# littlemesie/recommend-tf2.0

Measured on NVIDIA B200. Metric: DLRM train samples/sec, higher is better.
Workload: dtype f32

## Files before the change

### include/rtf_b200.h

```cpp
#ifndef RTF_B200_H
#define RTF_B200_H

#include <stddef.h>
#include <stdint.h>

#ifdef __cplusplus
extern "C" {
#endif

#define RTF_MAX_FIELDS 64

#define RTF_E_ARG (-1)
#define RTF_E_ALIGN (-2)
#define RTF_E_RANGE (-3)
#define RTF_E_WORKSPACE (-4)

enum { RTF_POOL_NONE = 0, RTF_POOL_SUM = 1, RTF_POOL_MEAN = 2,
       RTF_POOL_SKIP_INVALID = 0x100 };
enum { RTF_OPT_NONE = 0, RTF_OPT_SGD = 1, RTF_OPT_ADAGRAD = 2, RTF_OPT_ADAM = 3 };

typedef struct rtf_opt {
  int32_t kind;
  float lr;
  float beta1;
// ... 116 lines not shown
int rtf_din_attn_bwd(const float* d_q, int64_t q_sb, const float* d_k, int64_t k_sb,
                     const float* d_v, int64_t v_sb, const float* d_mask, int64_t m_sb,
                     const float* d_W, const float* d_bias, int act, int64_t B, int L, int d,
                     const float* d_gout, int64_t go_sb, float* d_gq, int64_t gq_sb, float* d_gk,
                     int64_t gk_sb, float* d_gv, int64_t gv_sb, float* d_gw_rows, void* stream);

int rtf_log_uniform_workspace(int S, size_t* bytes);
int rtf_log_uniform_sample(uint64_t seed, int S, int64_t range_max, int64_t* d_sampled,
                           int32_t* d_num_tries, void* d_ws, void* stream);
int rtf_log_uniform_sample_dseed(const uint64_t* d_seed, int S, int64_t range_max,
                                 int64_t* d_sampled, int32_t* d_num_tries, void* d_ws, void* stream);
int rtf_log_uniform_expected(const int64_t* d_ids, int64_t n, int64_t range_max,
                             const int32_t* d_num_tries, float* d_out, void* stream);
int rtf_sampled_softmax_workspace(int S, int D, size_t* bytes);
int rtf_sampled_softmax_fwd(const float* d_x, int64_t x_sb, const float* d_W, const float* d_bias,
                            const int64_t* d_labels, const int64_t* d_sampled,
                            const float* d_true_exp, const float* d_samp_exp, int64_t B, int64_t N,
                            int S, int D, int remove_hits, float* d_loss, float* d_lse, void* d_ws,
                            int32_t* d_err, void* stream);
int rtf_sampled_softmax_bwd(const float* d_x, int64_t x_sb, const float* d_W, const float* d_bias,
                            const int64_t* d_labels, const int64_t* d_sampled,
                            const float* d_true_exp, const float* d_samp_exp, int64_t B, int64_t N,
                            int S, int D, int remove_hits, const float* d_lse,
                            const float* d_gloss, float* d_gx, int64_t gx_sb, float* d_G,
                            void* d_ws, void* stream);

int rtf_ssm_gather(const float* d_W, const float* d_bias, const int64_t* d_sampled,
                   const float* d_samp_exp, int64_t N, int S, int D, float* d_Ws, float* d_cs,
                   int32_t* d_err, void* stream);
int rtf_ssm_logits_fwd(const float* d_logits, int64_t ld, const float* d_x, int64_t x_sb,
                       const float* d_W, const float* d_bias, const int64_t* d_labels,
                       const int64_t* d_sampled, const float* d_true_exp, const float* d_cs,
                       int64_t B, int64_t N, int S, int D, int remove_hits, float* d_loss,
                       float* d_lse, int32_t* d_err, void* stream);
int rtf_ssm_logits_bwd(const float* d_logits, int64_t ld, const float* d_x, int64_t x_sb,
                       const float* d_W, const float* d_bias, const int64_t* d_labels,
                       const int64_t* d_sampled, const float* d_true_exp, const float* d_cs,
                       int64_t B, int64_t N, int S, int D, int remove_hits, const float* d_lse,
                       const float* d_gloss, float* d_g0, float* d_G1, int64_t g1_ld, void* stream);
int rtf_ssm_true_gx(const float* d_W, const int64_t* d_labels, const float* d_g0, int64_t B,
                    int64_t N, int D, float* d_gx, int64_t gx_sb, void* stream);

int rtf_relu_bwd_colsum_workspace(int64_t B, int cols, size_t* bytes);
int rtf_relu_bwd_colsum(const float* d_gy, const float* d_y, int64_t B, int cols, float* d_g,
                        float* d_colsum, void* d_ws, void* stream);

int rtf_bce_workspace(int64_t n, size_t* bytes);
int rtf_bce_fwd(const float* d_y, const float* d_p, int64_t n, float* d_loss, float* d_dp,
                void* d_ws, void* stream);

int rtf_bn_workspace(int64_t B, int C, size_t* bytes);
int rtf_bn_fwd(const float* d_x, int64_t ldx, int64_t B, int C, const float* d_gamma,
               const float* d_beta, float eps, float momentum, float* d_y, int64_t ldy,
               float* d_mean, float* d_invstd, float* d_moving_mean, float* d_moving_var,
               void* d_ws, size_t ws_bytes, void* stream);
int rtf_bn_bwd(const float* d_dy, int64_t lddy, const float* d_x, int64_t ldx, int64_t B, int C,
               const float* d_mean, const float* d_invstd, const float* d_gamma, float* d_dx,
               int64_t lddx, float* d_dgamma, float* d_dbeta, void* d_ws, size_t ws_bytes,
               void* stream);

int rtf_layernorm_workspace(int64_t rows, int C, size_t* bytes);
int rtf_layernorm_fwd(const float* d_x, int64_t rows, int C, const float* d_gamma,
                      const float* d_beta, float eps, float* d_y, float* d_mean, float* d_rstd,
                      void* stream);
int rtf_layernorm_bwd(const float* d_dy, const float* d_x, const float* d_mean, const float* d_rstd,
                      const float* d_gamma, int64_t rows, int C, float* d_dx, float* d_dgamma,
                      float* d_dbeta, void* d_ws, size_t ws_bytes, void* stream);

int rtf_dense_gemm_nn_workspace(int M, int N, int K, int batch, size_t* bytes);
int rtf_dense_gemm_nt_workspace(int M, int N, int K, int batch, size_t* bytes);
int rtf_dense_gemm_tn_workspace(int M, int N, int K, int batch, size_t* bytes);
int rtf_dense_gemm_nn(const float* d_a, int64_t lda, int64_t stride_a, const float* d_b, int64_t ldb,
                      int64_t stride_b, const float* d_bias, int relu, float* d_out, int64_t ldd,
                      int64_t stride_d, int M, int N, int K, int batch, void* d_ws, size_t ws_bytes,
                      void* stream);
int rtf_dense_gemm_nt(const float* d_a, int64_t lda, int64_t stride_a, const float* d_b, int64_t ldb,
                      int64_t stride_b, const float* d_bias, int relu, float* d_out, int64_t ldd,
                      int64_t stride_d, int M, int N, int K, int batch, void* d_ws, size_t ws_bytes,
                      void* stream);
int rtf_dense_gemm_tn(const float* d_a, int64_t lda, int64_t stride_a, const float* d_b, int64_t ldb,
                      int64_t stride_b, const float* d_bias, int relu, float* d_out, int64_t ldd,
                      int64_t stride_d, int M, int N, int K, int batch, void* d_ws, size_t ws_bytes,
                      void* stream);

int rtf_autoint_layer_supported(int F, int dm, int H, int hs);
int rtf_autoint_layer_workspace(int64_t B, int dm, int HS, size_t* bytes);
int rtf_autoint_layer_fwd(const float* d_x, int64_t B, int F, int dm, const float* d_wq,
                          const float* d_wk, const float* d_wv, const float* d_w0, int H, int hs,
                          int act, float scale, float* d_out, void* stream);
int rtf_autoint_layer_bwd(const float* d_x, int64_t B, int F, int dm, const float* d_wq,
                          const float* d_wk, const float* d_wv, const float* d_w0, int H, int hs,
                          int act, float scale, const float* d_out, const float* d_gout,
                          float* d_gx, float* d_gw, void* d_ws, size_t ws_bytes, void* stream);

int rtf_sasrec_score_fwd(const float* d_info, int64_t info_sb, const float* d_pos_tab,
                         int64_t pos_rows, const float* d_neg_tab, int64_t neg_rows,
                         const void* d_pos_ids, const void* d_neg_ids, int ids_i64, int64_t neg_sb,
                         int64_t B, int NEG, int D, float* d_logits, float* d_loss_rows,
                         int32_t* d_err, void* stream);
int rtf_sasrec_score_bwd(const float* d_info, int64_t info_sb, const float* d_pos_tab,
                         int64_t pos_rows, const float* d_neg_tab, int64_t neg_rows,
                         const void* d_pos_ids, const void* d_neg_ids, int ids_i64, int64_t neg_sb,
                         int64_t B, int NEG, int D, const float* d_logits, const float* d_gloss,
                         const float* d_glogits, float* d_ginfo, float* d_gemb, void* stream);

int rtf_topk_ip_workspace(int64_t B, int64_t N, int D, int k, size_t* bytes);
int rtf_topk_ip(const float* d_users, int64_t u_ld, int64_t B, const float* d_items, int64_t i_ld,
                int64_t N, int D, int k, int64_t* d_out_idx, float* d_out_score, int32_t* d_flag,
                void* d_ws, size_t ws_bytes, void* stream);

int rtf_peer_pull_rows(const int64_t* d_peer_tab, const int64_t* d_peer_str, int64_t sample0, int G,
                       uint64_t rw_mask, const int64_t* rows, int n_fields, int D, const void* d_ids,
                       int ids_i64, int64_t B, int64_t ids_sb, int64_t ids_sf, float* d_out,
                       int64_t out_sb, int32_t* d_err, void* stream);

int rtf_dense_adam(float* d_w, const float* d_g, float* d_m, float* d_v, int64_t n,
                   const rtf_opt* opt, void* stream);
int rtf_rows_apply_dense(float* d_w, float* d_s1, float* d_s2, const float* d_g,
                         const float* d_touched, int64_t rows, int dim, const rtf_opt* opt,
                         void* stream);

#ifdef __cplusplus
}
#endif
#endif
```

### recommend-tf2.0_b200/_lib.py

```python
from __future__ import annotations

import ctypes as C
import os
import subprocess
import sys

_HERE = os.path.dirname(os.path.abspath(__file__))
LIB_PATH = os.path.join(_HERE, "librtf_b200.so")
CSRC_DIR = os.path.join(_HERE, "csrc")
HEADER_PATH = os.path.join(os.path.dirname(_HERE), "include", "rtf_b200.h")

POOL_NONE, POOL_SUM, POOL_MEAN = 0, 1, 2
OPT_NONE, OPT_SGD, OPT_ADAGRAD, OPT_ADAM = 0, 1, 2, 3
SEG_CHUNK = 64
MAX_FIELDS = 64


class RtfError(RuntimeError):
    pass


class rtf_opt(C.Structure):
    _fields_ = [("kind", C.c_int32), ("lr", C.c_float), ("beta1", C.c_float),
                ("beta2", C.c_float), ("eps", C.c_float), ("l2", C.c_float),
                ("lr_dev", C.c_void_p)]


_p = C.c_void_p
_i64 = C.c_int64
_int = C.c_int

SIGNATURES = {
    "rtf_version": [C.POINTER(C.c_int)],
    "rtf_embed_fwd": [_p, _p, _p, _int, _p, _int, _i64, _int, _i64, _i64, _i64, _int, _p, _i64,
                      _p, _p],
    "rtf_embed_bwd_workspace": [_i64, _int, C.POINTER(C.c_size_t)],
    "rtf_embed_bwd": [_p, _p, _p, _p, _p, _int, _p, _int, _p, _int, _i64, _int, _i64, _i64,
                      _i64, _int, _p, _i64, C.POINTER(rtf_opt), _p, _p, _p,
                      C.POINTER(C.c_int), _p, C.c_size_t, _p],
    "rtf_embed_bwd_prepare": [_p, _p, _int, _p, _int, _p, _int, _i64, _int, _i64, _i64, _i64, _p,
                              C.POINTER(C.c_int), _p, C.c_size_t, _p],
    "rtf_embed_bwd_apply": [_p, _p, _p, _p, _p, _int, _p, _int, _i64, _int, _int, _p, _i64,
                            C.POINTER(rtf_opt), _p, _p, _p, C.c_size_t, _p],
    "rtf_dot_interact_fwd": [_p, _i64, _int, _int, _p, _i64, _int, _p],
    "rtf_dot_interact_bwd": [_p, _p, _i64, _i64, _int, _int, _p, _p],
    "rtf_dot_rows_fwd": [_p, _p, _int, _int, _i64, _p, _i64, _int, _p, _i64, _p],
    "rtf_dot_rows_bwd": [_p, _p, _int, _int, _i64, _p, _i64, _p, _p, _p],
    "rtf_embed_dot_fwd": [_p, _p, _int, _int, _p, _int, _i64, _i64, _i64, _p, _i64, _p, _i64,
                          _int, _p, _p],
    "rtf_embed_dot_bwd": [_p, _p, _int, _int, _p, _int, _i64, _i64, _i64, _p, _i64, _p, _i64,
                          _p, _i64, _p, _i64, _p],
    "rtf_embed_dot_peer_fwd": [_p, _p, _i64, _int, C.c_uint64, _p, _int, _int, _p, _int, _i64, _i64, _i64, _p,
                               _i64, _p, _i64, _int, _p, _i64, _p, _p],
    "rtf_embed_dot_peer_bwd": [_p, _i64, _p, _int, _int, _p, _int, _i64, _i64, _i64, _p, _i64, _p,
                               _i64, _p, _i64, _p, _p, _int, C.c_uint64, _i64, _p],
    "rtf_colsum_workspace": [_i64, _int, C.POINTER(C.c_size_t)],
    "rtf_colsum": [_p, _i64, _p, _i64, _int, _p, _p, _p],
    "rtf_bn_workspace": [_i64, _int, C.POINTER(C.c_size_t)],
    "rtf_bn_fwd": [_p, _i64, _i64, _int, _p, _p, C.c_float, C.c_float, _p, _i64, _p, _p, _p, _p, _p,
                   C.c_size_t, _p],
    "rtf_bn_bwd": [_p, _i64, _p, _i64, _i64, _int, _p, _p, _p, _p, _i64, _p, _p, _p, C.c_size_t, _p],
    "rtf_layernorm_workspace": [_i64, _int, C.POINTER(C.c_size_t)],
    "rtf_layernorm_fwd": [_p, _i64, _int, _p, _p, C.c_float, _p, _p, _p, _p],
    "rtf_layernorm_bwd": [_p, _p, _p, _p, _p, _i64, _int, _p, _p, _p, _p, C.c_size_t, _p],
    "rtf_bce_workspace": [_i64, C.POINTER(C.c_size_t)],
    "rtf_bce_fwd": [_p, _p, _i64, _p, _p, _p, _p],
    "rtf_relu_bwd_colsum_workspace": [_i64, _int, C.POINTER(C.c_size_t)],
    "rtf_relu_bwd_colsum": [_p, _p, _i64, _int, _p, _p, _p, _p],
    "rtf_autoint_layer_supported": [_int, _int, _int, _int],
    "rtf_autoint_layer_workspace": [_i64, _int, _int, C.POINTER(C.c_size_t)],
    "rtf_autoint_layer_fwd": [_p, _i64, _int, _int, _p, _p, _p, _p, _int, _int, _int, C.c_float, _p, _p],
    "rtf_autoint_layer_bwd": [_p, _i64, _int, _int, _p, _p, _p, _p, _int, _int, _int, C.c_float, _p, _p,
                              _p, _p, _p, C.c_size_t, _p],
    "rtf_sasrec_score_fwd": [_p, _i64, _p, _i64, _p, _i64, _p, _p, _int, _i64, _i64, _int, _int, _p, _p, _p, _p],
    "rtf_sasrec_score_bwd": [_p, _i64, _p, _i64, _p, _i64, _p, _p, _int, _i64, _i64, _int, _int, _p, _p, _p,
                             _p, _p, _p],
    "rtf_topk_ip_workspace": [_i64, _i64, _int, _int, C.POINTER(C.c_size_t)],
    "rtf_topk_ip": [_p, _i64, _i64, _p, _i64, _i64, _int, _int, _p, _p, _p, _p, C.c_size_t, _p],
    "rtf_peer_pull_rows": [_p, _p, _i64, _int, C.c_uint64, _p, _int, _int, _p, _int, _i64, _i64, _i64, _p,
                           _i64, _p, _p],
    "rtf_ssm_gather": [_p, _p, _p, _p, _i64, _int, _int, _p, _p, _p, _p],
    "rtf_ssm_logits_fwd": [_p, _i64, _p, _i64, _p, _p, _p, _p, _p, _p, _i64, _i64, _int, _int, _int, _p, _p,
                           _p, _p],
    "rtf_ssm_logits_bwd": [_p, _i64, _p, _i64, _p, _p, _p, _p, _p, _p, _i64, _i64, _int, _int, _int, _p, _p,
                           _p, _p, _i64, _p],
    "rtf_ssm_true_gx": [_p, _p, _p, _i64, _i64, _int, _p, _i64, _p],
    "rtf_dense_adam": [_p, _p, _p, _p, _i64, C.POINTER(rtf_opt), _p],
    "rtf_rows_apply_dense": [_p, _p, _p, _p, _p, _i64, _int, C.POINTER(rtf_opt), _p],
    "rtf_dense_gemm_nn_workspace": [_int, _int, _int, _int, C.POINTER(C.c_size_t)],
    "rtf_dense_gemm_nt_workspace": [_int, _int, _int, _int, C.POINTER(C.c_size_t)],
    "rtf_dense_gemm_tn_workspace": [_int, _int, _int, _int, C.POINTER(C.c_size_t)],
    "rtf_dense_gemm_nn": [_p, _i64, _i64, _p, _i64, _i64, _p, _int, _p, _i64, _i64, _int, _int, _int,
                          _int, _p, C.c_size_t, _p],
    "rtf_dense_gemm_nt": [_p, _i64, _i64, _p, _i64, _i64, _p, _int, _p, _i64, _i64, _int, _int, _int,
                          _int, _p, C.c_size_t, _p],
    "rtf_dense_gemm_tn": [_p, _i64, _i64, _p, _i64, _i64, _p, _int, _p, _i64, _i64, _int, _int, _int,
                          _int, _p, C.c_size_t, _p],
    "rtf_fm_layer_workspace": [_i64, _int, C.POINTER(C.c_size_t)],
    "rtf_fm_layer_fwd": [_p, _i64, _p, _int, _p, _i64, _int, _int, _i64, _int, _int, _p, _p, _p],
    "rtf_fm_layer_bwd": [_p, _i64, _p, _int, _p, _i64, _int, _int, _i64, _int, _int, _p, _p,
                         _i64, _p, _p, _i64, _p, _p],
    "rtf_fm_gather_fwd": [_p, _p, _int, _int, _int, _p, _int, _p, _i64, _p, _int, _i64, _i64,
                          _i64, _p, _p, _p, _p, _p],
    "rtf_fm_gather_bwd": [_p, _p, _int, _int, _int, _p, _int, _p, _i64, _p, _int, _i64, _i64,
                          _i64, _p, _p, _p, _p, _p, _p, _p],
    "rtf_attn_fwd": [_p, _i64, _i64, _p, _i64, _i64, _p, _i64, _i64, _p, _i64, _p, _i64, _int,
                     _int, _int, _int, _int, _int, C.c_float, _p, _i64, _i64, _p, _p, _p],
    "rtf_attn_bwd": [_p, _i64, _i64, _p, _i64, _i64, _p, _i64, _i64, _p, _i64, _p, _i64, _int,
                     _int, _int, _int, _int, _int, C.c_float, _p, _i64, _i64, _p, _p, _p, _i64,
                     _i64, _p, _p, _i64, _i64, _p, _i64, _i64, _p, _i64, _i64, _p],
    "rtf_din_attn_fwd": [_p, _i64, _p, _i64, _p, _i64, _p, _i64, _p, _p, _int, _i64, _int, _int,
                         _p, _i64, _p],
    "rtf_din_attn_bwd": [_p, _i64, _p, _i64, _p, _i64, _p, _i64, _p, _p, _int, _i64, _int, _int,
                         _p, _i64, _p, _i64, _p, _i64, _p, _i64, _p, _p],
    "rtf_log_uniform_workspace": [_int, C.POINTER(C.c_size_t)],
    "rtf_log_uniform_sample": [C.c_uint64, _int, _i64, _p, _p, _p, _p],
    "rtf_log_uniform_sample_dseed": [_p, _int, _i64, _p, _p, _p, _p],
    "rtf_log_uniform_expected": [_p, _i64, _i64, _p, _p, _p],
    "rtf_sampled_softmax_workspace": [_int, _int, C.POINTER(C.c_size_t)],
    "rtf_sampled_softmax_fwd": [_p, _i64, _p, _p, _p, _p, _p, _p, _i64, _i64, _int, _int, _int,
                                _p, _p, _p, _p, _p],
    "rtf_sampled_softmax_bwd": [_p, _i64, _p, _p, _p, _p, _p, _p, _i64, _i64, _int, _int, _int,
                                _p, _p, _p, _i64, _p, _p, _p],
}

_lib = None


def build(verbose: bool = False) -> str:
    cmd = ["make", "-C", CSRC_DIR, "-j", str(min(8, os.cpu_count() or 1))]
    res = subprocess.run(cmd, stdout=subprocess.PIPE, stderr=subprocess.STDOUT, text=True)
    if verbose or res.returncode != 0:
        sys.stderr.write(res.stdout)
    if res.returncode != 0:
        raise RtfError("building librtf_b200.so failed (see make output above)")
    return LIB_PATH


def lib() -> C.CDLL:
    global _lib
    if _lib is None:
        if not os.path.exists(LIB_PATH):
            raise RtfError(
                f"{LIB_PATH} not found: run `python -c 'import __graft_entry__ as g; g.build()'` "
                "(or make -C recommend-tf2.0_b200/csrc). There is no CPU fallback.")
        handle = C.CDLL(LIB_PATH)
        for name, argtypes in SIGNATURES.items():
            fn = getattr(handle, name)
            fn.argtypes = argtypes
            fn.restype = C.c_int
        _lib = handle
    return _lib


def check(rc: int, what: str) -> None:
    if rc == 0:
        return
    if rc < 0:
        names = {-1: "RTF_E_ARG", -2: "RTF_E_ALIGN", -3: "RTF_E_RANGE", -4: "RTF_E_WORKSPACE"}
        raise RtfError(f"{what}: {names.get(rc, rc)}")
    raise RtfError(f"{what}: cudaError_t {rc}")


def require_cuda(t, what: str):
    if not t.is_cuda:
        raise RtfError(f"{what}: tensor is on {t.device}; the recommend-tf2.0_b200 kernels run "
                       "on CUDA (sm_100a) only and have no CPU fallback")


def current_stream_ptr() -> int:
    import torch
    try:
        return torch._C._cuda_getCurrentRawStream(torch._C._cuda_getDevice())
    except AttributeError:
        return torch.cuda.current_stream().cuda_stream


def host_array(ctype, values):
    arr = (ctype * len(values))(*values)
    return arr
# ... 1 lines not shown
```

### recommend-tf2.0_b200/core.py

```python
from __future__ import annotations

import math
import os
from typing import Callable, Optional, Sequence

import torch
import torch.nn.functional as F


class Layer(torch.nn.Module):

    def __init__(self, name: Optional[str] = None, **kwargs):
        super().__init__()
        self._built = False
        self._name = name

    def build(self, input_shape):
        pass

    def call(self, inputs, **kwargs):
        raise NotImplementedError

    def forward(self, inputs, *args, **kwargs):
        if not self._built:
# ... 178 lines not shown
    if buf is None or buf.numel() < nbytes:
        buf = _SCRATCH[key] = torch.empty(max(nbytes, 1 << 20), dtype=torch.uint8, device=device)
    return buf


def _wgrad_splits(B: int, kin: int, n: int, clusters: int = 74) -> int:
    tiles = ((kin + 255) // 256) * ((n + 127) // 128)
    best, best_eff = 1, 0.0
    s = 1
    while s <= 64 and B % s == 0 and (B // s) % 4 == 0 and B // s >= 512:
        waves = tiles * s / clusters
        eff = waves / -(-tiles * s // clusters)
        if eff > best_eff + 0.02:
            best, best_eff = s, eff
        s *= 2
    return best


def _wgrad(x: torch.Tensor, g: torch.Tensor) -> torch.Tensor:
    B = x.shape[0]
    if B >= 1024 and _x6_ok(x, g):
        return dense_gemm("tn", x, g, splits=_wgrad_splits(B, x.shape[1], g.shape[1]))
    S = 16
    if B >= 8192 and B % S == 0 and x.is_contiguous() and g.is_contiguous():
        return torch.bmm(x.view(S, B // S, -1).transpose(1, 2), g.view(S, B // S, -1)).sum(0)
    return x.t() @ g


def _relu_bwd_bias_grad(gy: torch.Tensor, y):
    B, N = gy.shape
    if gy.is_cuda and N % 4 == 0 and B > 0:
        import ctypes as C
        from . import _lib as L
        gy = gy.contiguous()
        key = ("relu_bwd", B, N)
        if key not in _GEMM_WS_BYTES:
            nb = C.c_size_t(0)
            L.check(L.lib().rtf_relu_bwd_colsum_workspace(B, N, C.byref(nb)), "rtf_relu_bwd_colsum_workspace")
            _GEMM_WS_BYTES[key] = max(nb.value, 16)
        ws = _scratch(_GEMM_WS_BYTES[key], gy.device)
        g = torch.empty_like(gy) if y is not None else gy
        db = torch.empty(N, dtype=torch.float32, device=gy.device)
        L.check(L.lib().rtf_relu_bwd_colsum(gy.data_ptr(), None if y is None else y.data_ptr(), B, N,
                                            g.data_ptr(), db.data_ptr(), ws.data_ptr(),
                                            L.current_stream_ptr()), "rtf_relu_bwd_colsum")
        return g, db
    g = torch.ops.aten.threshold_backward(gy, y, 0.0) if y is not None else gy.contiguous()
    return g, g.sum(0)


class _DenseFn(torch.autograd.Function):

    @staticmethod
    def forward(ctx, x, w, b, relu):
        kpad = 0
        if (x.shape[1] % 4 and DENSE_GEMM == "bf16x6" and x.is_cuda and x.shape[0] >= 1024
                and w.shape[1] % 4 == 0 and x.shape[0] % 4 == 0):
            kpad = (-x.shape[1]) % 4
            x = F.pad(x, (0, kpad))
            w = F.pad(w, (0, 0, 0, kpad))
        ctx.kpad = kpad
        if x.shape[0] >= 1024 and _x6_ok(x, w) and b.data_ptr() % 16 == 0:
            y = dense_gemm("nn", x, w, b, relu)
        else:
            y = torch._addmm_activation(b, x, w, use_gelu=False) if relu else torch.addmm(b, x, w)
        ctx.save_for_backward(x, w, y if relu else None)
        ctx.relu = relu
        return y

    @staticmethod
    def backward(ctx, gy):
        x, w, y = ctx.saved_tensors
        g, gb = _relu_bwd_bias_grad(gy, y if ctx.relu else None)
        gx = None
        if ctx.needs_input_grad[0]:
            gx = dense_gemm("nt", g, w) if (g.shape[0] >= 1024 and _x6_ok(g, w)) else g @ w.t()
        gw = _wgrad(x, g) if ctx.needs_input_grad[1] else None
        if ctx.kpad:
            gx = None if gx is None else gx[:, : gx.shape[1] - ctx.kpad].contiguous()
            gw = None if gw is None else gw[: gw.shape[0] - ctx.kpad]
        return gx, gw, gb, None


class _BatchNormTrainFn(torch.autograd.Function):

    @staticmethod
    def forward(ctx, x2, gamma, beta, eps, momentum, moving_mean, moving_var):
        import ctypes as C
        from . import _lib as L
        L.require_cuda(x2, "BatchNormalization(x)")
        if x2.dtype != torch.float32:
            raise TypeError("BatchNormalization: fp32 activations only")
        if x2.stride(1) != 1:
            x2 = x2.contiguous()
        B, Cc = x2.shape
        key = ("bn", B, Cc)
        if key not in _GEMM_WS_BYTES:
            nb = C.c_size_t(0)
            L.check(L.lib().rtf_bn_workspace(B, Cc, C.byref(nb)), "rtf_bn_workspace")
            _GEMM_WS_BYTES[key] = nb.value
        ws = _scratch(_GEMM_WS_BYTES[key], x2.device)
        y = torch.empty((B, Cc), dtype=torch.float32, device=x2.device)
        stats = torch.empty((2, Cc), dtype=torch.float32, device=x2.device)
        L.check(L.lib().rtf_bn_fwd(x2.data_ptr(), x2.stride(0), B, Cc,
                                   None if gamma is None else gamma.data_ptr(),
                                   None if beta is None else beta.data_ptr(), eps, momentum,
                                   y.data_ptr(), y.stride(0), stats[0].data_ptr(), stats[1].data_ptr(),
                                   None if moving_mean is None else moving_mean.data_ptr(),
                                   None if moving_var is None else moving_var.data_ptr(),
                                   ws.data_ptr(), ws.numel(), L.current_stream_ptr()), "rtf_bn_fwd")
        ctx.save_for_backward(x2, stats, gamma)
        ctx.has_beta = beta is not None
        return y

    @staticmethod
    def backward(ctx, dy):
        import ctypes as C
        from . import _lib as L
        x2, stats, gamma = ctx.saved_tensors
        B, Cc = x2.shape
        if dy.stride(1) != 1:
            dy = dy.contiguous()
        ws = _scratch(_GEMM_WS_BYTES[("bn", B, Cc)], x2.device)
        dx = torch.empty_like(dy) if ctx.needs_input_grad[0] else None
        dg = torch.empty(Cc, dtype=torch.float32, device=dy.device) if gamma is not None else None
        db = torch.empty(Cc, dtype=torch.float32, device=dy.device) if ctx.has_beta else None
        L.check(L.lib().rtf_bn_bwd(dy.data_ptr(), dy.stride(0), x2.data_ptr(), x2.stride(0), B, Cc,
                                   stats[0].data_ptr(), stats[1].data_ptr(),
                                   None if gamma is None else gamma.data_ptr(),
                                   None if dx is None else dx.data_ptr(),
                                   0 if dx is None else dx.stride(0),
                                   None if dg is None else dg.data_ptr(),
                                   None if db is None else db.data_ptr(),
                                   ws.data_ptr(), ws.numel(), L.current_stream_ptr()), "rtf_bn_bwd")
        return dx, dg, db, None, None, None, None


class BatchNormalization(Layer):

    def __init__(self, center: bool = True, scale: bool = True, momentum: float = 0.99,
                 epsilon: float = 1e-3, trainable: bool = True, **kwargs):
        super().__init__(**kwargs)
        self.center, self.scale, self.momentum, self.epsilon = center, scale, momentum, epsilon

    def build(self, input_shape):
        c = input_shape[-1]
        self.gamma = self.add_weight("gamma", (c,), "ones") if self.scale else None
        self.beta = self.add_weight("beta", (c,), "zeros") if self.center else None
        dev = _default_device()
        self.register_buffer("moving_mean", torch.zeros(c, device=dev))
        self.register_buffer("moving_variance", torch.ones(c, device=dev))

    def call(self, x, **kwargs):
        shp = x.shape
        x2 = x.reshape(-1, shp[-1])
        if self.training and x2.is_cuda and x2.shape[0] > 0:
            y = _BatchNormTrainFn.apply(x2, self.gamma, self.beta, self.epsilon, self.momentum,
                                        self.moving_mean, self.moving_variance)
        elif self.training:
            y, mean, invstd = torch.native_batch_norm(x2, self.gamma, self.beta, None, None, True, 0.0,
                                                      self.epsilon)
            with torch.no_grad():
                var = 1.0 / (invstd * invstd) - self.epsilon
                self.moving_mean.mul_(self.momentum).add_(mean, alpha=1.0 - self.momentum)
                self.moving_variance.mul_(self.momentum).add_(var, alpha=1.0 - self.momentum)
        else:
            y = F.batch_norm(x2, self.moving_mean, self.moving_variance, self.gamma, self.beta,
                             False, 0.0, self.epsilon)
        return y.reshape(shp)


class Dropout(Layer):
    def __init__(self, rate: float = 0.0, **kwargs):
        super().__init__(**kwargs)
        self.rate = rate

    def call(self, x, **kwargs):
        return F.dropout(x, self.rate, self.training) if self.rate > 0 else x


class DNN(Layer):

    def __init__(self, hidden_units: Sequence[int], activation="relu", dnn_dropout: float = 0.0,
                 input_bn: bool = True, **kwargs):
        super().__init__(**kwargs)
        self.dnn_network = torch.nn.ModuleList([Dense(u, activation=activation) for u in hidden_units])
        self.dropout = Dropout(dnn_dropout)
        self.bn = BatchNormalization() if input_bn else None

    def call(self, inputs, **kwargs):
        x = inputs
        if self.bn is not None:
            x = self.bn(x)
        for dnn in self.dnn_network:
            x = dnn(x)
        return self.dropout(x)


class DenseAdam:

    ALIGN = 64

    def __init__(self, params, lr: float = 1e-3, beta1: float = 0.9, beta2: float = 0.999,
                 eps: float = 1e-7):
        from . import _lib as L
        params = [p for p in params if p.requires_grad]
        if not params:
            raise ValueError("DenseAdam: no trainable parameters")
        for p in params:
            L.require_cuda(p, "DenseAdam(param)")
            if p.dtype != torch.float32:
                raise TypeError("DenseAdam: fp32 parameters only")
        self.params, self.lr, self.beta1, self.beta2, self.eps = params, lr, beta1, beta2, eps
        self.t = 0
        self.lr_dev = None
        offs, n = [], 0
        for p in params:
            offs.append(n)
            n += (p.numel() + self.ALIGN - 1) // self.ALIGN * self.ALIGN
        dev = params[0].device
        self.flat = torch.zeros(n, dtype=torch.float32, device=dev)
        self.flat_grad = torch.zeros_like(self.flat)
        self.m = torch.zeros_like(self.flat)
        self.v = torch.zeros_like(self.flat)
        with torch.no_grad():
            for p, o in zip(params, offs):
                view = self.flat[o:o + p.numel()].view(p.shape)
                view.copy_(p.data)
                p.data = view
                p.grad = self.flat_grad[o:o + p.numel()].view(p.shape)
        self.offsets = offs

    def zero_grad(self):
        self.flat_grad.zero_()
        for p, o in zip(self.params, self.offsets):
            if p.grad is None or p.grad.data_ptr() != self.flat_grad.data_ptr() + 4 * o:
                p.grad = self.flat_grad[o:o + p.numel()].view(p.shape)

    def lr_for_step(self, t: int) -> float:
        return self.lr * math.sqrt(1.0 - self.beta2 ** t) / (1.0 - self.beta1 ** t)

    def enable_device_lr(self):
        if self.lr_dev is None:
            self.lr_dev = torch.zeros(1, dtype=torch.float32, device=self.flat.device)
            self.lr_dev.fill_(self.lr_for_step(max(self.t, 1)))

    def advance(self):
        self.t += 1
        if self.lr_dev is not None:
            self.lr_dev.fill_(self.lr_for_step(self.t))

    def apply(self):
        import ctypes as C
        from . import _lib as L
        st = L.rtf_opt(L.OPT_ADAM, self.lr_for_step(max(self.t, 1)), self.beta1, self.beta2,
                       self.eps, 0.0, None if self.lr_dev is None else self.lr_dev.data_ptr())
        L.check(L.lib().rtf_dense_adam(self.flat.data_ptr(), self.flat_grad.data_ptr(),
                                       self.m.data_ptr(), self.v.data_ptr(), self.flat.numel(),
                                       C.byref(st), L.current_stream_ptr()), "rtf_dense_adam")

    def step(self):
        self.advance()
        self.apply()


def _tree_map(fn, x):
    if isinstance(x, torch.Tensor):
        return fn(x)
    if isinstance(x, (list, tuple)):
        return type(x)(_tree_map(fn, v) for v in x)
    if isinstance(x, dict):
        return {k: _tree_map(fn, v) for k, v in x.items()}
    return x


def _tree_leaves(x, out=None):
    out = [] if out is None else out
    if isinstance(x, torch.Tensor):
# ... 90 lines not shown
```

### recommend-tf2.0_b200/csrc/dense_gemm.cuh

```cuda
#pragma once
#include <cfloat>
#include <cstdint>
#include <cuda_runtime.h>

#include "cute/tensor.hpp"
#include "cutlass/cutlass.h"
#include "cutlass/epilogue/collective/collective_builder.hpp"
#include "cutlass/epilogue/fusion/operations.hpp"
#include "cutlass/epilogue/thread/activation.h"
#include "cutlass/gemm/collective/collective_builder.hpp"
#include "cutlass/gemm/device/gemm_universal_adapter.h"
#include "cutlass/gemm/kernel/gemm_universal.hpp"
#include "cutlass/numeric_types.h"

#include "rtf_b200.h"

namespace rtf_gemm {

using namespace cute;

using RowMajor = cutlass::layout::RowMajor;
using ColumnMajor = cutlass::layout::ColumnMajor;

template <class LayoutA, class LayoutB, int Bands, class MmaTile = Shape<_256, _128, _32>,
          class Cluster = Shape<_2, _1, _1>,
          class MainSchedule = cutlass::gemm::KernelTmaWarpSpecialized2SmFastFP32SmemSm100,
          class EpiSchedule = cutlass::epilogue::TmaWarpSpecialized2Sm, class ElementC = void,
          int PromotionInterval = 2, class AccCopyAtom = void>
struct FastF32Gemm {
  using Arch = cutlass::arch::Sm100;
  using OpClass = cutlass::arch::OpClassTensorOp;
  using Fusion = cutlass::epilogue::fusion::LinCombPerColBiasEltAct<
      cutlass::epilogue::thread::Clamp, float, float, float, ElementC, float>;
  using Epilogue = typename cutlass::epilogue::collective::CollectiveBuilder<
      Arch, OpClass, MmaTile, Cluster, cutlass::epilogue::collective::EpilogueTileAuto, float,
      float, ElementC, RowMajor, 4, float, RowMajor, 4, EpiSchedule, Fusion>::CollectiveOp;
  using Stock = typename cutlass::gemm::collective::CollectiveBuilder<
      Arch, OpClass, float, LayoutA, 4, float, LayoutB, 4, float, MmaTile, Cluster,
      cutlass::gemm::collective::StageCountAutoCarveout<static_cast<int>(
          sizeof(typename Epilogue::SharedStorage))>,
      MainSchedule>::CollectiveOp;
  using SP = typename Stock::DispatchPolicy;
  using Policy = cutlass::gemm::MainloopSm100TmaUmmaWarpSpecializedFastF32<
      SP::Load2TransformPipelineStageCount, SP::Transform2MmaPipelineStageCount,
      SP::Schedule::SchedulerPipelineStageCount, SP::Schedule::AccumulatorPipelineStageCount, Bands,
      SP::ScalingFactor, (PromotionInterval > 0 ? PromotionInterval : SP::AccPromotionInterval),
      typename SP::ClusterShape,
      cute::conditional_t<cute::is_void_v<AccCopyAtom>, typename SP::AccumulatorCopyAtom, AccCopyAtom>,
      typename SP::ArchTag>;
  using Mainloop = cutlass::gemm::collective::CollectiveMma<
      Policy, typename Stock::TileShape, float, typename Stock::StrideA, float,
      typename Stock::StrideB, typename Stock::TiledMma, typename Stock::GmemTiledCopyA,
      typename Stock::SmemLayoutAtomsA, typename Stock::CopyAtomsA, typename Stock::TransformA,
      typename Stock::GmemTiledCopyB, typename Stock::SmemLayoutAtomsB, typename Stock::CopyAtomsB,
      typename Stock::TransformB>;
  using Kernel = cutlass::gemm::kernel::GemmUniversal<Shape<int, int, int, int>, Mainloop, Epilogue>;
  using Gemm = cutlass::gemm::device::GemmUniversalAdapter<Kernel>;
  using StrideA = typename Kernel::StrideA;
  using StrideB = typename Kernel::StrideB;
  using StrideD = typename Kernel::StrideD;

  template <class Stride, bool KContiguous>
  static Stride make_stride(int64_t ld, int64_t batch) {
    Stride s{};
    if constexpr (KContiguous) {
      get<0>(s) = ld;
    } else {
      get<1>(s) = ld;
    }
    get<2>(s) = batch;
    return s;
  }

  static typename Gemm::Arguments make_args(const float* A, int64_t lda, int64_t sA, const float* B,
                                            int64_t ldb, int64_t sB, const float* bias, float lo,
                                            float hi, float* D, int64_t ldd, int64_t sD, int M, int N,
                                            int K, int batch) {
    constexpr bool a_k = std::is_same_v<LayoutA, RowMajor>;
    constexpr bool b_k = std::is_same_v<LayoutB, ColumnMajor>;
    StrideA sa = make_stride<StrideA, a_k>(lda, sA);
    StrideB sb = make_stride<StrideB, b_k>(ldb, sB);
    StrideD sd = make_stride<StrideD, true>(ldd, sD);
    typename Gemm::Arguments args{cutlass::gemm::GemmUniversalMode::kGemm,
                                  {M, N, K, batch},
                                  {A, sa, B, sb},
                                  {{}, nullptr, sd, D, sd}};
    args.epilogue.thread.alpha = 1.f;
    args.epilogue.thread.beta = 0.f;
    args.epilogue.thread.bias_ptr = bias;
    args.epilogue.thread.activation.lower_bound = lo;
    args.epilogue.thread.activation.upper_bound = hi;
    static int sm_count = 0;
    int dev = 0;
    cudaGetDevice(&dev);
    if (sm_count == 0) cudaDeviceGetAttribute(&sm_count, cudaDevAttrMultiProcessorCount, dev);
    args.hw_info.device_id = dev;
    args.hw_info.sm_count = sm_count;
    return args;
  }

  static int workspace(int M, int N, int K, int batch, size_t* bytes) {
    auto args = make_args(nullptr, K, 0, nullptr, K, 0, nullptr, 0.f, 0.f, nullptr, N, 0, M, N, K, batch);
    *bytes = Gemm::get_workspace_size(args);
    return 0;
  }

  static int run(const float* A, int64_t lda, int64_t sA, const float* B, int64_t ldb, int64_t sB,
                 const float* bias, int relu, float* D, int64_t ldd, int64_t sD, int M, int N, int K,
                 int batch, void* ws, size_t ws_bytes, cudaStream_t st) {
    if (!A || !B || !D || M <= 0 || N <= 0 || K <= 0 || batch <= 0) return RTF_E_ARG;
    if (lda % 4 || ldb % 4 || ldd % 4 || sA % 4 || sB % 4 || sD % 4 || (uintptr_t)A % 16 ||
        (uintptr_t)B % 16 || (uintptr_t)D % 16 || (uintptr_t)bias % 16)
      return RTF_E_ALIGN;
    const float lo = relu ? 0.f : -INFINITY, hi = INFINITY;
    auto args = make_args(A, lda, sA, B, ldb, sB, bias, lo, hi, D, ldd, sD, M, N, K, batch);
    Gemm gemm;
    if (gemm.can_implement(args) != cutlass::Status::kSuccess) return RTF_E_RANGE;
    if (Gemm::get_workspace_size(args) > ws_bytes) return RTF_E_WORKSPACE;
    if (gemm.initialize(args, ws, st) != cutlass::Status::kSuccess) return RTF_E_ARG;
    cutlass::Status s = gemm.run(st);
    if (s != cutlass::Status::kSuccess) return (int)cudaGetLastError() ? (int)cudaGetLastError() : RTF_E_ARG;
    return 0;
  }
};

}
```

### recommend-tf2.0_b200/csrc/dense_gemm_nn.cu

```cuda
#include "dense_gemm.cuh"

using G = rtf_gemm::FastF32Gemm<rtf_gemm::RowMajor, rtf_gemm::RowMajor, RTF_GEMM_BANDS>;

extern "C" int rtf_dense_gemm_nn_workspace(int M, int N, int K, int batch, size_t* bytes) {
  if (!bytes) return RTF_E_ARG;
  return G::workspace(M, N, K, batch, bytes);
}

extern "C" int rtf_dense_gemm_nn(const float* d_a, int64_t lda, int64_t stride_a, const float* d_b,
                                 int64_t ldb, int64_t stride_b, const float* d_bias, int relu,
                                 float* d_out, int64_t ldd, int64_t stride_d, int M, int N, int K,
                                 int batch, void* d_ws, size_t ws_bytes, void* stream) {
  return G::run(d_a, lda, stride_a, d_b, ldb, stride_b, d_bias, relu, d_out, ldd, stride_d, M, N, K,
                batch, d_ws, ws_bytes, (cudaStream_t)stream);
}
```

### recommend-tf2.0_b200/csrc/dense_gemm_nt.cu

```cuda
#include "dense_gemm.cuh"

using G = rtf_gemm::FastF32Gemm<rtf_gemm::RowMajor, rtf_gemm::ColumnMajor, RTF_GEMM_BANDS>;

extern "C" int rtf_dense_gemm_nt_workspace(int M, int N, int K, int batch, size_t* bytes) {
  if (!bytes) return RTF_E_ARG;
  return G::workspace(M, N, K, batch, bytes);
}

extern "C" int rtf_dense_gemm_nt(const float* d_a, int64_t lda, int64_t stride_a, const float* d_b,
                                 int64_t ldb, int64_t stride_b, const float* d_bias, int relu,
                                 float* d_out, int64_t ldd, int64_t stride_d, int M, int N, int K,
                                 int batch, void* d_ws, size_t ws_bytes, void* stream) {
  return G::run(d_a, lda, stride_a, d_b, ldb, stride_b, d_bias, relu, d_out, ldd, stride_d, M, N, K,
                batch, d_ws, ws_bytes, (cudaStream_t)stream);
}
```

Measured before the change: 8.848 million.

## Fuse ReLU mask into MLP stack GEMM epilogues for forward and backward

Adds a custom autograd function for a stack of ReLU dense layers. The forward GEMM epilogue writes a packed 1-bit ReLU mask, and the backward data-grad GEMM epilogue applies that mask. This removes a separate elementwise ReLU-backward pass that re-reads the saved activations, and it adds two new CUTLASS epilogue visitor nodes. The costs are more code and the fixed layout constraints for the fused path (N divisible by 128, batch at least 1024, bf16x6 mode).

Result: faster. 9.106 million (median of 6 runs) (+2.9%).

```diff
diff --git a/include/rtf_b200.h b/include/rtf_b200.h
--- a/include/rtf_b200.h
+++ b/include/rtf_b200.h
@@ -222,6 +222,12 @@
                       int64_t stride_b, const float* d_bias, int relu, float* d_out, int64_t ldd,
                       int64_t stride_d, int M, int N, int K, int batch, void* d_ws, size_t ws_bytes,
                       void* stream);
+int rtf_dense_gemm_nn_relu_mask(const float* d_a, int64_t lda, const float* d_b, int64_t ldb,
+                                const float* d_bias, float* d_out, int64_t ldd, uint32_t* d_mask, int M,
+                                int N, int K, void* d_ws, size_t ws_bytes, void* stream);
+int rtf_dense_gemm_nt_masked(const float* d_a, int64_t lda, const float* d_b, int64_t ldb,
+                             const uint32_t* d_mask, float* d_out, int64_t ldd, int M, int N, int K,
+                             void* d_ws, size_t ws_bytes, void* stream);
 
 int rtf_autoint_layer_supported(int F, int dm, int H, int hs);
 int rtf_autoint_layer_workspace(int64_t B, int dm, int HS, size_t* bytes);
diff --git a/recommend-tf2.0_b200/_lib.py b/recommend-tf2.0_b200/_lib.py
--- a/recommend-tf2.0_b200/_lib.py
+++ b/recommend-tf2.0_b200/_lib.py
@@ -96,6 +96,8 @@
                           _int, _p, C.c_size_t, _p],
     "rtf_dense_gemm_tn": [_p, _i64, _i64, _p, _i64, _i64, _p, _int, _p, _i64, _i64, _int, _int, _int,
                           _int, _p, C.c_size_t, _p],
+    "rtf_dense_gemm_nn_relu_mask": [_p, _i64, _p, _i64, _p, _p, _i64, _p, _int, _int, _int, _p, C.c_size_t, _p],
+    "rtf_dense_gemm_nt_masked": [_p, _i64, _p, _i64, _p, _p, _i64, _int, _int, _int, _p, C.c_size_t, _p],
     "rtf_fm_layer_workspace": [_i64, _int, C.POINTER(C.c_size_t)],
     "rtf_fm_layer_fwd": [_p, _i64, _p, _int, _p, _i64, _int, _int, _i64, _int, _int, _p, _p, _p],
     "rtf_fm_layer_bwd": [_p, _i64, _p, _int, _p, _i64, _int, _int, _i64, _int, _int, _p, _p,
diff --git a/recommend-tf2.0_b200/core.py b/recommend-tf2.0_b200/core.py
--- a/recommend-tf2.0_b200/core.py
+++ b/recommend-tf2.0_b200/core.py
@@ -284,6 +284,98 @@
         return gx, gw, gb, None
 
 
+def _dense_gemm_mask(kind: str, a: torch.Tensor, b: torch.Tensor, bias=None, mask=None):
+    import ctypes as C
+    from . import _lib as L
+    lib = L.lib()
+    M, K = a.shape
+    N = b.shape[1] if kind == "nn" else b.shape[0]
+    key = (kind, M, N, K, 1)
+    if key not in _GEMM_WS_BYTES:
+        nb = C.c_size_t(0)
+        L.check(getattr(lib, f"rtf_dense_gemm_{kind}_workspace")(M, N, K, 1, C.byref(nb)),
+                f"rtf_dense_gemm_{kind}_workspace")
+        _GEMM_WS_BYTES[key] = max(nb.value, 16)
+    ws = _scratch(_GEMM_WS_BYTES[key], a.device)
+    out = torch.empty((M, N), dtype=torch.float32, device=a.device)
+    if kind == "nn":
+        mask = torch.empty(((M + 31) // 32, N // 32, 32), dtype=torch.int32, device=a.device)
+        L.check(lib.rtf_dense_gemm_nn_relu_mask(a.data_ptr(), a.stride(0), b.data_ptr(), b.stride(0),
+                                                bias.data_ptr(), out.data_ptr(), N, mask.data_ptr(), M, N, K,
+                                                ws.data_ptr(), ws.numel(), L.current_stream_ptr()),
+                "rtf_dense_gemm_nn_relu_mask")
+        return out, mask
+    L.check(lib.rtf_dense_gemm_nt_masked(a.data_ptr(), a.stride(0), b.data_ptr(), b.stride(0),
+                                         mask.data_ptr(), out.data_ptr(), N, M, N, K, ws.data_ptr(),
+                                         ws.numel(), L.current_stream_ptr()), "rtf_dense_gemm_nt_masked")
+    return out
+
+
+def _stack_ok(layers, x: torch.Tensor) -> bool:
+    if not (len(layers) >= 2 and torch.is_grad_enabled() and DENSE_GEMM == "bf16x6" and x.is_cuda
+            and x.dim() == 2 and x.dtype == torch.float32 and x.shape[0] >= 1024 and x.shape[0] % 4 == 0):
+        return False
+    if x.shape[1] % 4 == 0 and not (x.is_contiguous() and x.data_ptr() % 16 == 0):
+        return False
+    for i, d in enumerate(layers):
+        if d._act_name != "relu" or d.bias is None or d.units % 4:
+            return False
+        if i + 1 < len(layers) and d.units % 128:
+            return False
+        if not (d.kernel.is_cuda and d.kernel.dtype == torch.float32 and d.kernel.is_contiguous()
+                and d.bias.is_contiguous() and d.kernel.data_ptr() % 16 == 0 and d.bias.data_ptr() % 16 == 0):
+            return False
+    return layers[0].kernel.shape[0] == x.shape[1]
+
+
+class _DenseStackFn(torch.autograd.Function):
+
+    @staticmethod
+    def forward(ctx, x, *wb):
+        n = len(wb) // 2
+        ws, bs = wb[0::2], wb[1::2]
+        kpad = (-x.shape[1]) % 4
+        w0 = ws[0]
+        if kpad:
+            x = F.pad(x, (0, kpad))
+            w0 = F.pad(w0, (0, 0, 0, kpad))
+        xs, masks = [x], []
+        h = x
+        for i in range(n):
+            w = w0 if i == 0 else ws[i]
+            if i + 1 < n:
+                h, m = _dense_gemm_mask("nn", h, w, bs[i])
+                masks.append(m)
+            else:
+                h = dense_gemm("nn", h, w, bs[i], True)
+            xs.append(h)
+        ctx.kpad, ctx.n = kpad, n
+        ctx.save_for_backward(*xs, w0, *ws[1:], *masks)
+        return h
+
+    @staticmethod
+    def backward(ctx, gy):
+        n = ctx.n
+        saved = ctx.saved_tensors
+        xs, ws, masks = saved[: n + 1], saved[n + 1: 2 * n + 1], saved[2 * n + 1:]
+        g, gb = _relu_bwd_bias_grad(gy, xs[n])
+        grads = [None] * (2 * n)
+        gx = None
+        for i in range(n - 1, -1, -1):
+            grads[2 * i + 1] = gb
+            if ctx.needs_input_grad[1 + 2 * i]:
+                grads[2 * i] = _wgrad(xs[i], g)
+            if i > 0:
+                g = _dense_gemm_mask("nt", g.contiguous(), ws[i], mask=masks[i - 1])
+                g, gb = _relu_bwd_bias_grad(g, None)
+            elif ctx.needs_input_grad[0]:
+                gx = dense_gemm("nt", g, ws[0])
+        if ctx.kpad:
+            gx = None if gx is None else gx[:, : gx.shape[1] - ctx.kpad].contiguous()
+            grads[0] = None if grads[0] is None else grads[0][: grads[0].shape[0] - ctx.kpad]
+        return (gx, *grads)
+
+
 class _BatchNormTrainFn(torch.autograd.Function):
 
     @staticmethod
@@ -394,8 +486,19 @@
         x = inputs
         if self.bn is not None:
             x = self.bn(x)
-        for dnn in self.dnn_network:
-            x = dnn(x)
+        layers = list(self.dnn_network)
+        fan_in = x.shape[-1]
+        for d in layers:
+            if not d._built:
+                d.build((None, fan_in))
+                d._built = True
+            fan_in = d.units
+        if _stack_ok(layers, x):
+            wb = [t for d in layers for t in (d.kernel, d.bias)]
+            x = _DenseStackFn.apply(x, *wb)
+        else:
+            for dnn in layers:
+                x = dnn(x)
         return self.dropout(x)
 
 
diff --git a/recommend-tf2.0_b200/csrc/dense_gemm.cuh b/recommend-tf2.0_b200/csrc/dense_gemm.cuh
--- a/recommend-tf2.0_b200/csrc/dense_gemm.cuh
+++ b/recommend-tf2.0_b200/csrc/dense_gemm.cuh
@@ -22,19 +22,166 @@
 using RowMajor = cutlass::layout::RowMajor;
 using ColumnMajor = cutlass::layout::ColumnMajor;
 
+constexpr int kMaskAlign = 128;
+
+enum EpiMode { kEpiPlain = 0, kEpiReluMaskOut = 1, kEpiMaskIn = 2 };
+
+namespace fus = cutlass::epilogue::fusion;
+
+template <class Word>
+struct MaskNodeBase {
+  struct SharedStorage {};
+  struct Arguments {
+    Word* ptr_mask = nullptr;
+  };
+  using Params = Arguments;
+
+  template <class ProblemShape>
+  static constexpr Params to_underlying_arguments(ProblemShape const&, Arguments const& a, void*) {
+    return a;
+  }
+  template <class ProblemShape>
+  static bool can_implement(ProblemShape const&, Arguments const& a) {
+    return a.ptr_mask != nullptr;
+  }
+  template <class ProblemShape>
+  static size_t get_workspace_size(ProblemShape const&, Arguments const&) {
+    return 0;
+  }
+  template <class ProblemShape>
+  static cutlass::Status initialize_workspace(ProblemShape const&, Arguments const&, void*, cudaStream_t,
+                                              cutlass::CudaHostAdapter* = nullptr) {
+    return cutlass::Status::kSuccess;
+  }
+
+  CUTLASS_HOST_DEVICE MaskNodeBase() {}
+  CUTLASS_HOST_DEVICE MaskNodeBase(Params const& p, SharedStorage const&) : params(p) {}
+  Params const params;
+
+  CUTLASS_DEVICE bool is_producer_load_needed() const { return false; }
+  CUTLASS_DEVICE bool is_C_load_needed() const { return false; }
+  template <class... Args>
+  CUTLASS_DEVICE auto get_producer_load_callbacks(fus::ProducerLoadArgs<Args...> const&) {
+    return fus::EmptyProducerLoadCallbacks{};
+  }
+
+  CUTLASS_DEVICE static int64_t word(int row, int col, int ld) {
+    return ((int64_t)(row >> 5) * (ld >> 5) + (col >> 5)) * 32 + (row & 31);
+  }
+};
+
+template <class Args>
+CUTLASS_DEVICE auto first_element(Args const& args) {
+  auto [M, N, K, L] = args.problem_shape_mnkl;
+  return cute::make_tuple(int(M) - int(get<0>(args.residue_tCcD)), int(N) - int(get<1>(args.residue_tCcD)),
+                          int(M), int(N));
+}
+
+struct ReluMaskStore : MaskNodeBase<uint32_t> {
+  using MaskNodeBase<uint32_t>::MaskNodeBase;
+
+  template <class CTensor, class Residue>
+  struct ConsumerStoreCallbacks : fus::EmptyConsumerStoreCallbacks {
+    CUTLASS_DEVICE ConsumerStoreCallbacks(CTensor c, Residue res, int m0, int n0, int rows, int ld, uint32_t* p)
+        : tC_cD(c), residue(res), m0(m0), n0(n0), rows(rows), ld(ld), mask(p) {}
+    CTensor tC_cD;
+    Residue residue;
+    int m0, n0, rows, ld;
+    uint32_t* mask;
+
+    template <class ElementAccumulator, int F>
+    CUTLASS_DEVICE cutlass::Array<float, F> visit(cutlass::Array<ElementAccumulator, F> const&, int epi_v,
+                                                  int epi_m, int epi_n, cutlass::Array<float, F> const& y) {
+      static_assert(F == 32, "a fragment is one mask word: 32 columns of one row");
+      auto c = tC_cD(_, _, _, epi_m, epi_n)(epi_v * F);
+      const int row = m0 + get<0>(c), col = n0 + get<1>(c);
+      uint32_t w = 0;
+      CUTLASS_PRAGMA_UNROLL
+      for (int i = 0; i < F; ++i) w |= uint32_t(y[i] > 0.f) << i;
+      if (row < rows && col < ld) mask[MaskNodeBase::word(row, col, ld)] = w;
+      return y;
+    }
+  };
+
+  template <bool ReferenceSrc, class... Args>
+  CUTLASS_DEVICE auto get_consumer_store_callbacks(fus::ConsumerStoreArgs<Args...> const& args) {
+    auto [m0, n0, M, N] = first_element(args);
+    return ConsumerStoreCallbacks<decltype(args.tCcD), decltype(args.residue_tCcD)>(
+        args.tCcD, args.residue_tCcD, m0, n0, M, N, params.ptr_mask);
+  }
+};
+
+struct MaskSelect : MaskNodeBase<const uint32_t> {
+  using MaskNodeBase<const uint32_t>::MaskNodeBase;
+  static constexpr int kWords = 4;
+
+  template <class CTensor, class Residue>
+  struct ConsumerStoreCallbacks : fus::EmptyConsumerStoreCallbacks {
+    CUTLASS_DEVICE ConsumerStoreCallbacks(CTensor c, Residue res, int m0, int n0, int rows, int ld,
+                                          const uint32_t* p)
+        : tC_cD(c), residue(res), m0(m0), n0(n0), rows(rows), ld(ld), mask(p) {}
+    CTensor tC_cD;
+    Residue residue;
+    int m0, n0, rows, ld;
+    const uint32_t* mask;
+    uint32_t w[kWords];
+
+    CUTLASS_DEVICE void begin() {
+      CUTLASS_PRAGMA_UNROLL
+      for (int q = 0; q < kWords; ++q)
+        w[q] = (m0 < rows && n0 + 32 * q < ld) ? mask[MaskNodeBase::word(m0, n0 + 32 * q, ld)] : 0u;
+    }
+
+    template <class ElementAccumulator, int F>
+    CUTLASS_DEVICE cutlass::Array<float, F> visit(cutlass::Array<ElementAccumulator, F> const&, int epi_v,
+                                                  int epi_m, int epi_n, cutlass::Array<float, F> const& y) {
+      static_assert(F == 32, "a fragment is one mask word: 32 columns of one row");
+      auto c = tC_cD(_, _, _, epi_m, epi_n)(epi_v * F);
+      const int q = get<1>(c) >> 5;
+      uint32_t bits = w[0];
+      CUTLASS_PRAGMA_UNROLL
+      for (int k = 1; k < kWords; ++k) bits = q == k ? w[k] : bits;
+      cutlass::Array<float, F> out;
+      CUTLASS_PRAGMA_UNROLL
+      for (int i = 0; i < F; ++i) out[i] = (bits >> i) & 1u ? y[i] : 0.f;
+      return out;
+    }
+  };
+
+  template <bool ReferenceSrc, class... Args>
+  CUTLASS_DEVICE auto get_consumer_store_callbacks(fus::ConsumerStoreArgs<Args...> const& args) {
+    static_assert(decltype(size<1>(shape(args.tCcD)))::value == 1 &&
+                  decltype(size<3>(shape(args.tCcD)))::value == 1,
+                  "one accumulator row per thread and epilogue tile");
+    auto [m0, n0, M, N] = first_element(args);
+    return ConsumerStoreCallbacks<decltype(args.tCcD), decltype(args.residue_tCcD)>(
+        args.tCcD, args.residue_tCcD, m0, n0, M, N, params.ptr_mask);
+  }
+};
+
 template <class LayoutA, class LayoutB, int Bands, class MmaTile = Shape<_256, _128, _32>,
           class Cluster = Shape<_2, _1, _1>,
           class MainSchedule = cutlass::gemm::KernelTmaWarpSpecialized2SmFastFP32SmemSm100,
           class EpiSchedule = cutlass::epilogue::TmaWarpSpecialized2Sm, class ElementC = void,
-          int PromotionInterval = 2, class AccCopyAtom = void>
+          int PromotionInterval = 2, class AccCopyAtom = void, int Mode = kEpiPlain>
 struct FastF32Gemm {
   using Arch = cutlass::arch::Sm100;
   using OpClass = cutlass::arch::OpClassTensorOp;
   using Fusion = cutlass::epilogue::fusion::LinCombPerColBiasEltAct<
       cutlass::epilogue::thread::Clamp, float, float, float, ElementC, float>;
-  using Epilogue = typename cutlass::epilogue::collective::CollectiveBuilder<
+  template <class F>
+  using EpilogueOf = typename cutlass::epilogue::collective::CollectiveBuilder<
       Arch, OpClass, MmaTile, Cluster, cutlass::epilogue::collective::EpilogueTileAuto, float,
-      float, ElementC, RowMajor, 4, float, RowMajor, 4, EpiSchedule, Fusion>::CollectiveOp;
+      float, ElementC, RowMajor, 4, float, RowMajor, 4, EpiSchedule, F>::CollectiveOp;
+  using PlainEpilogue = EpilogueOf<Fusion>;
+  using PlainTree = typename PlainEpilogue::FusionCallbacks;
+  using Callbacks = cute::conditional_t<
+      Mode == kEpiPlain, Fusion,
+      cute::conditional_t<Mode == kEpiReluMaskOut, fus::Sm90EVT<ReluMaskStore, PlainTree>,
+                          fus::Sm90EVT<MaskSelect, PlainTree>>>;
+  using Epilogue = EpilogueOf<Callbacks>;
+  static_assert(std::is_same_v<typename Epilogue::EpilogueTile, typename PlainEpilogue::EpilogueTile>);
+  static_assert(sizeof(typename Epilogue::SharedStorage) == sizeof(typename PlainEpilogue::SharedStorage));
   using Stock = typename cutlass::gemm::collective::CollectiveBuilder<
       Arch, OpClass, float, LayoutA, 4, float, LayoutB, 4, float, MmaTile, Cluster,
       cutlass::gemm::collective::StageCountAutoCarveout<static_cast<int>(
@@ -48,6 +195,11 @@
       typename SP::ClusterShape,
       cute::conditional_t<cute::is_void_v<AccCopyAtom>, typename SP::AccumulatorCopyAtom, AccCopyAtom>,
       typename SP::ArchTag>;
+  using PlainSP = typename FastF32Gemm<LayoutA, LayoutB, Bands, MmaTile, Cluster, MainSchedule, EpiSchedule,
+                                       ElementC, PromotionInterval, AccCopyAtom, kEpiPlain>::SP;
+  static_assert(SP::Load2TransformPipelineStageCount == PlainSP::Load2TransformPipelineStageCount &&
+                SP::Transform2MmaPipelineStageCount == PlainSP::Transform2MmaPipelineStageCount,
+                "a mask epilogue must not cost the mainloop a pipeline stage");
   using Mainloop = cutlass::gemm::collective::CollectiveMma<
       Policy, typename Stock::TileShape, float, typename Stock::StrideA, float,
       typename Stock::StrideB, typename Stock::TiledMma, typename Stock::GmemTiledCopyA,
@@ -75,7 +227,7 @@
   static typename Gemm::Arguments make_args(const float* A, int64_t lda, int64_t sA, const float* B,
                                             int64_t ldb, int64_t sB, const float* bias, float lo,
                                             float hi, float* D, int64_t ldd, int64_t sD, int M, int N,
-                                            int K, int batch) {
+                                            int K, int batch, const uint32_t* mask = nullptr) {
     constexpr bool a_k = std::is_same_v<LayoutA, RowMajor>;
     constexpr bool b_k = std::is_same_v<LayoutB, ColumnMajor>;
     StrideA sa = make_stride<StrideA, a_k>(lda, sA);
@@ -85,11 +237,20 @@
                                   {M, N, K, batch},
                                   {A, sa, B, sb},
                                   {{}, nullptr, sd, D, sd}};
-    args.epilogue.thread.alpha = 1.f;
-    args.epilogue.thread.beta = 0.f;
-    args.epilogue.thread.bias_ptr = bias;
-    args.epilogue.thread.activation.lower_bound = lo;
-    args.epilogue.thread.activation.upper_bound = hi;
+    auto& plain = [&]() -> auto& {
+      if constexpr (Mode == kEpiPlain) return args.epilogue.thread;
+      else return args.epilogue.thread.op_0;
+    }();
+    plain.alpha = 1.f;
+    plain.beta = 0.f;
+    plain.bias_ptr = bias;
+    plain.activation.lower_bound = lo;
+    plain.activation.upper_bound = hi;
+    if constexpr (Mode == kEpiReluMaskOut) {
+      args.epilogue.thread.op_1 = {const_cast<uint32_t*>(mask)};
+    } else if constexpr (Mode == kEpiMaskIn) {
+      args.epilogue.thread.op_1 = {mask};
+    }
     static int sm_count = 0;
     int dev = 0;
     cudaGetDevice(&dev);
@@ -107,13 +268,17 @@
 
   static int run(const float* A, int64_t lda, int64_t sA, const float* B, int64_t ldb, int64_t sB,
                  const float* bias, int relu, float* D, int64_t ldd, int64_t sD, int M, int N, int K,
-                 int batch, void* ws, size_t ws_bytes, cudaStream_t st) {
+                 int batch, void* ws, size_t ws_bytes, cudaStream_t st, const uint32_t* mask = nullptr) {
     if (!A || !B || !D || M <= 0 || N <= 0 || K <= 0 || batch <= 0) return RTF_E_ARG;
     if (lda % 4 || ldb % 4 || ldd % 4 || sA % 4 || sB % 4 || sD % 4 || (uintptr_t)A % 16 ||
         (uintptr_t)B % 16 || (uintptr_t)D % 16 || (uintptr_t)bias % 16)
       return RTF_E_ALIGN;
+    if constexpr (Mode != kEpiPlain) {
+      if (!mask || batch != 1) return RTF_E_ARG;
+      if (N % kMaskAlign || (uintptr_t)mask % 16) return RTF_E_ALIGN;
+    }
     const float lo = relu ? 0.f : -INFINITY, hi = INFINITY;
-    auto args = make_args(A, lda, sA, B, ldb, sB, bias, lo, hi, D, ldd, sD, M, N, K, batch);
+    auto args = make_args(A, lda, sA, B, ldb, sB, bias, lo, hi, D, ldd, sD, M, N, K, batch, mask);
     Gemm gemm;
     if (gemm.can_implement(args) != cutlass::Status::kSuccess) return RTF_E_RANGE;
     if (Gemm::get_workspace_size(args) > ws_bytes) return RTF_E_WORKSPACE;
@@ -124,4 +289,10 @@
   }
 };
 
+template <class LayoutA, class LayoutB, int Bands, int Mode>
+using FastF32GemmMask =
+    FastF32Gemm<LayoutA, LayoutB, Bands, Shape<_256, _128, _32>, Shape<_2, _1, _1>,
+                cutlass::gemm::KernelTmaWarpSpecialized2SmFastFP32SmemSm100,
+                cutlass::epilogue::TmaWarpSpecialized2Sm, void, 2, void, Mode>;
+
 }
diff --git a/recommend-tf2.0_b200/csrc/dense_gemm_nn.cu b/recommend-tf2.0_b200/csrc/dense_gemm_nn.cu
--- a/recommend-tf2.0_b200/csrc/dense_gemm_nn.cu
+++ b/recommend-tf2.0_b200/csrc/dense_gemm_nn.cu
@@ -14,3 +14,14 @@
   return G::run(d_a, lda, stride_a, d_b, ldb, stride_b, d_bias, relu, d_out, ldd, stride_d, M, N, K,
                 batch, d_ws, ws_bytes, (cudaStream_t)stream);
 }
+
+using GMaskOut = rtf_gemm::FastF32GemmMask<rtf_gemm::RowMajor, rtf_gemm::RowMajor, RTF_GEMM_BANDS,
+                                              rtf_gemm::kEpiReluMaskOut>;
+
+extern "C" int rtf_dense_gemm_nn_relu_mask(const float* d_a, int64_t lda, const float* d_b, int64_t ldb,
+                                           const float* d_bias, float* d_out, int64_t ldd,
+                                           uint32_t* d_mask, int M, int N, int K, void* d_ws,
+                                           size_t ws_bytes, void* stream) {
+  return GMaskOut::run(d_a, lda, 0, d_b, ldb, 0, d_bias, 1, d_out, ldd, 0, M, N, K, 1, d_ws, ws_bytes,
+                       (cudaStream_t)stream, d_mask);
+}
diff --git a/recommend-tf2.0_b200/csrc/dense_gemm_nt.cu b/recommend-tf2.0_b200/csrc/dense_gemm_nt.cu
--- a/recommend-tf2.0_b200/csrc/dense_gemm_nt.cu
+++ b/recommend-tf2.0_b200/csrc/dense_gemm_nt.cu
@@ -14,3 +14,13 @@
   return G::run(d_a, lda, stride_a, d_b, ldb, stride_b, d_bias, relu, d_out, ldd, stride_d, M, N, K,
                 batch, d_ws, ws_bytes, (cudaStream_t)stream);
 }
+
+using GMaskIn = rtf_gemm::FastF32GemmMask<rtf_gemm::RowMajor, rtf_gemm::ColumnMajor, RTF_GEMM_BANDS,
+                                             rtf_gemm::kEpiMaskIn>;
+
+extern "C" int rtf_dense_gemm_nt_masked(const float* d_a, int64_t lda, const float* d_b, int64_t ldb,
+                                        const uint32_t* d_mask, float* d_out, int64_t ldd, int M, int N,
+                                        int K, void* d_ws, size_t ws_bytes, void* stream) {
+  return GMaskIn::run(d_a, lda, 0, d_b, ldb, 0, nullptr, 0, d_out, ldd, 0, M, N, K, 1, d_ws, ws_bytes,
+                      (cudaStream_t)stream, d_mask);
+}
```
